# t-kychen/GaussianProcess-MCMC

Measured on NVIDIA B200. Metric: GP log-lik evals/sec (N=4096, batched chains), higher is better.
Workload: dtype f64

## Files before the change

### gaussianprocess-mcmc_b200/csrc/capi.cu

```cuda
#include "common.cuh"
#include "sequences.cuh"
#include "../../include/gpmc.h"

#include <stdarg.h>
#include <string.h>
#include <mutex>
#include <algorithm>
#include <vector>

namespace gpmc {

static thread_local char g_err[1024] = "";
static std::recursive_mutex g_api_mutex;
ApiLock::ApiLock() { g_api_mutex.lock(); }
ApiLock::~ApiLock() { g_api_mutex.unlock(); }
void set_error(const char *fmt, ...)
{
    va_list ap;
    va_start(ap, fmt);
    vsnprintf(g_err, sizeof(g_err), fmt, ap);
    va_end(ap);
}

struct EventPair { cudaEvent_t a, b; };
// ... 271 lines not shown
    if (failed.empty()) return 0;

    BatchView Bk{backup, (long long)N * ld, ld, nullptr, nullptr};
    { int rc0 = diag_stats(Bk, N, mean_dev, bad_dev, B, s); if (rc0) return rc0; }
    std::vector<double> mean(B);
    std::vector<int> bad(B);
    GPMC_CUDA_CHECK(cudaMemcpyAsync(mean.data(), mean_dev, B * sizeof(double), cudaMemcpyDeviceToHost, s));
    GPMC_CUDA_CHECK(cudaMemcpyAsync(bad.data(), bad_dev, B * sizeof(int), cudaMemcpyDeviceToHost, s));
    GPMC_CUDA_CHECK(cudaStreamSynchronize(s));
    std::vector<double> jit(B, 0.0);
    std::vector<int> todo;
    for (int i : failed) {
        if (bad[i]) info[i] = GPMC_INFO_NOT_PD;
        else { jit[i] = mean[i] * 1e-6; todo.push_back(i); }
    }
    for (int attempt = 0; attempt < 5 && !todo.empty(); ++attempt) {
        const int nf = (int)todo.size();
        GPMC_CUDA_CHECK(cudaMemcpyAsync(map_dev, todo.data(), nf * sizeof(int), cudaMemcpyHostToDevice, s));
        GPMC_CUDA_CHECK(cudaMemcpyAsync(jit_dev, jit.data(), B * sizeof(double), cudaMemcpyHostToDevice, s));
        BatchView Am{A_dev, (long long)N * ld, ld, map_dev, nullptr};
        restore_jitter_kernel<<<dim3(64, nf), 256, 0, s>>>(Am, backup, N, jit_dev);
        GPMC_LAUNCH_CHECK();
        for (int i : todo) info[i] = 0;
        GPMC_CUDA_CHECK(cudaMemcpyAsync(info_dev, info.data(), B * sizeof(int), cudaMemcpyHostToDevice, s));
        rc = potrf_sequence(Am, N, nf, info_dev, W, NB * NB, 0, zero_upper, s);
        if (rc) return rc;
        GPMC_CUDA_CHECK(cudaMemcpyAsync(info.data(), info_dev, B * sizeof(int), cudaMemcpyDeviceToHost, s));
        GPMC_CUDA_CHECK(cudaStreamSynchronize(s));
        std::vector<int> still;
        for (int i : todo) if (info[i] != 0) { still.push_back(i); jit[i] *= 10.0; }
        todo.swap(still);
    }
    for (int i : todo) info[i] = GPMC_INFO_NOT_PD;
    GPMC_CUDA_CHECK(cudaMemcpyAsync(info_dev, info.data(), B * sizeof(int), cudaMemcpyHostToDevice, s));
    GPMC_CUDA_CHECK(cudaStreamSynchronize(s));
    return 0;
}

int gpmc_loglik_batched(const double *x_dev, int N, int D, const double *g_dev, const double *hyp_dev, int B, int P,
                        int kind, int jitter_policy, double *loglik_dev, int *info_dev, void *ws_dev, size_t ws_bytes,
                        void *stream)
{
    GPMC_API_LOCK();
    cudaStream_t s = (cudaStream_t)stream;
    const int n_ell = (kind == GPMC_KIND_SE_ARD) ? D : 1;
    if (N <= 0 || D <= 0 || B < 0 || P != n_ell + 2) { set_error("loglik: bad shape N=%d D=%d B=%d P=%d kind=%d", N, D, B, P, kind); return GPMC_EINVAL; }
    if (B == 0) return 0;
    const LoglikLayout l = loglik_layout(N, B);
    if (!ws_dev || ws_bytes < l.fixed_bytes + l.per_item_bytes) {
        set_error("loglik: workspace %zu bytes cannot hold one item (%zu needed)", ws_bytes, l.fixed_bytes + l.per_item_bytes);
        return GPMC_ENOMEM;
    }
    char *wp = (char *)ws_dev;
    double *jit_dev = (double *)wp; wp += align_up((size_t)B * sizeof(double), 256);
    int *map_dev = (int *)wp; wp += align_up((size_t)B * sizeof(int), 256);
    int *band_dev = (int *)wp; wp += 256;
    double *xbox = (double *)wp;
    wp += align_up((size_t)32 * l.ld * sizeof(double), 256);
    const size_t wave_cap = std::min<size_t>((ws_bytes - l.fixed_bytes) / l.per_item_bytes, (size_t)MAX_BATCH_ITEMS);
    const int wave = (int)std::min<size_t>(wave_cap, (size_t)B);
    g_last_W = 0;
    g_last_waves = (B + wave - 1) / wave;
    { int rc0 = fill_int(info_dev, 0, B, s); if (rc0) return rc0; }

    if (wave < B && band_compact_allowed() && envelope_enabled() && band_enabled()) {
        const int nblk = env_blocks(N);
        const size_t wenv = align_up((size_t)B * nblk * sizeof(int), 256);
        char *cp = wp;
        int *w_all = (int *)cp; cp += wenv;
        int *env_all = (int *)cp; cp += wenv;
        const size_t room = ws_bytes - l.fixed_bytes;
        if (2 * wenv + 256 < room) {
            GPMC_CUDA_CHECK(cudaMemsetAsync(band_dev, 0, 2 * sizeof(int), s));
            int rc = launch_band_bound(x_dev, N, D, hyp_dev, P, n_ell, B, w_all, nblk, band_dev, xbox, s);
            if (rc) return rc;
            int bh[2] = {0, 0};
            GPMC_CUDA_CHECK(cudaMemcpyAsync(bh, band_dev, sizeof(bh), cudaMemcpyDeviceToHost, s));
            GPMC_CUDA_CHECK(cudaStreamSynchronize(s));
            const int Wc = (int)align_up((size_t)BAND_ROWS + (size_t)ENV_ROWS * bh[1], 16);
            const size_t per_item = (size_t)N * Wc * sizeof(double) + (size_t)l.ld * sizeof(double) + (size_t)NB * NB * sizeof(double);
            const size_t wave_c = std::min<size_t>((room - 2 * wenv - 256) / per_item, (size_t)MAX_BATCH_ITEMS);
            const int waves_c = wave_c > 0 ? (int)((B + wave_c - 1) / wave_c) : 0;
            const int nb_lo = waves_c > 0 ? B / waves_c : 0, nb_hi = waves_c > 0 ? (B + waves_c - 1) / waves_c : 0;
            if (Wc < l.ld && waves_c > 0 && waves_c < g_last_waves && potrf_compact_ok(N, nb_lo, 1) && potrf_compact_ok(N, nb_hi, 1)) {
                double *border = (double *)cp; cp += align_up((size_t)nb_hi * l.ld * sizeof(double), 256);
                double *Wsc = (double *)cp; cp += (size_t)nb_hi * NB * NB * sizeof(double);
                double *mats_c = (double *)cp;
                g_last_W = Wc;
                g_last_waves = waves_c;
                for (int wi = 0, s0 = 0; wi < waves_c; ++wi) {
                    const int nb = nb_lo + (wi < B % waves_c ? 1 : 0);
                    BatchView A{mats_c, (long long)N * Wc, Wc, nullptr, nullptr, Wc, N, border, l.ld};
                    const Envelope env{env_all + (size_t)s0 * nblk, nblk, N, bh[0]};
                    const Band band{w_all + (size_t)s0 * nblk, nblk, bh[1], 0};
                    const double *hyp_w = hyp_dev + (size_t)s0 * P;
                    const double *g_w = g_dev + (size_t)s0 * N;
                    int *info_w = info_dev + s0;
                    auto fill = [&](BatchView V, int nitems, const double *jit) -> int {
                        int rc = launch_cov_assemble(x_dev, N, D, hyp_w, P, n_ell, GPMC_ASM_ADD_S | GPMC_ASM_LOWER_ONLY, jit, V, nitems, s, env, band);
                        if (rc) return rc;
                        return border_set(V, N, g_w, N, nitems, s);
                    };
                    auto diag = [&](const double *h) { return host_diag_value(h, n_ell); };
                    rc = factor_wave(fill, diag, A, N, nb, hyp_w, P, info_w, Wsc, jit_dev, map_dev, jitter_policy, 1, s, 0, env);
                    if (rc) return rc;
                    if ((rc = border_finish(A, N, loglik_dev + s0, info_w, nb, s, 0))) return rc;
                    s0 += nb;
                }
                return 0;
            }
        }
    }

    double *mats = (double *)wp;
    double *W = (double *)(wp + (size_t)wave * l.mat_elems * sizeof(double));
    const Envelope env_ws{(int *)(W + (size_t)wave * NB * NB), env_blocks(N), N};
    int *band_w = env_ws.blk + (size_t)wave * env_blocks(N);
    ClearJoin clear{s};

    for (int s0 = 0; s0 < B; s0 += wave) {
        const int nb = std::min(wave, B - s0);
        const double *hyp_w = hyp_dev + (size_t)s0 * P;
        const double *g_w = g_dev + (size_t)s0 * N;
        int *info_w = info_dev + s0;
        BatchView A{mats, (long long)l.mat_elems, l.ld, nullptr, nullptr};
        const int fuse = potrf_fuse_auto(N, nb, 1);
        Envelope env = (envelope_enabled() && !fuse) ? env_ws : Envelope{};
        Band band{};
        int rc = 0;
        if (env.blk && band_enabled()) {
            const int mode = band_clear_mode();
            if (clear.pending) {
                GPMC_CUDA_CHECK(cudaStreamWaitEvent(s, clear.cs->done, 0));
                clear.pending = false;
            }
            GPMC_CUDA_CHECK(cudaMemsetAsync(band_dev, 0, 2 * sizeof(int), s));
            rc = launch_band_bound(x_dev, N, D, hyp_w, P, n_ell, nb, band_w, env_blocks(N), band_dev, xbox, s);
            if (rc) return rc;
            int bh[2] = {-1, 0};
            if (mode != 2 || (long long)nb * ((N + NB - 1) / NB) >= 1024) {
                GPMC_CUDA_CHECK(cudaMemcpyAsync(bh, band_dev, sizeof(bh), cudaMemcpyDeviceToHost, s));
                GPMC_CUDA_CHECK(cudaStreamSynchronize(s));
            }
            env.band = bh[0];
            band = Band{band_w, env_blocks(N), bh[1], mode == 2};
            if (mode == 1) {
                ClearStream *cs = clear.cs ? clear.cs : (clear.cs = clear_stream());
                if (!cs) { set_error("loglik: the band clear stream could not be created"); return GPMC_EINVAL; }
                GPMC_CUDA_CHECK(cudaEventRecord(cs->start, s));
                GPMC_CUDA_CHECK(cudaStreamWaitEvent(cs->s, cs->start, 0));
                BatchView Aw{mats, (long long)l.mat_elems, l.ld, nullptr, nullptr};
                if ((rc = launch_band_clear(Aw, N, band, nb, cs->s))) return rc;
                GPMC_CUDA_CHECK(cudaEventRecord(cs->done, cs->s));
                clear.pending = true;
            }
        }
        auto fill = [&](BatchView V, int nitems, const double *jit) -> int {
            int rc = launch_cov_assemble(x_dev, N, D, hyp_w, P, n_ell, GPMC_ASM_ADD_S | GPMC_ASM_LOWER_ONLY, jit, V, nitems, s, env, band);
            if (rc) return rc;
            return border_set(V, N, g_w, N, nitems, s);
        };
        auto diag = [&](const double *h) { return host_diag_value(h, n_ell); };
        rc = factor_wave(fill, diag, A, N, nb, hyp_w, P, info_w, W, jit_dev, map_dev, jitter_policy, 1, s, fuse, env);
        if (rc) return rc;
        rc = border_finish(A, N, loglik_dev + s0, info_w, nb, s, fuse);
        if (rc) return rc;
    }
    return 0;
}

struct HostPath {
    cudaStream_t stream = nullptr;
    void *dev = nullptr;  size_t dev_bytes = 0;
    void *ws = nullptr;   size_t ws_bytes = 0;
    void *pin = nullptr;  size_t pin_bytes = 0;
};
static HostPath g_hp;

static int ensure(void **p, size_t *have, size_t need, bool pinned)
{
    if (*have >= need) return 0;
    if (*p) { if (pinned) cudaFreeHost(*p); else cudaFree(*p); *p = nullptr; *have = 0; }
    cudaError_t e = pinned ? cudaMallocHost(p, need) : cudaMalloc(p, need);
    if (e != cudaSuccess) { set_error("allocation of %zu bytes failed: %s", need, cudaGetErrorString(e)); return (int)e; }
    *have = need;
    return 0;
}
// ... 147 lines not shown
```

### gaussianprocess-mcmc_b200/csrc/common.cuh

```cuda
#pragma once
#include <cuda_runtime.h>
#include <stdint.h>
#include <stdio.h>
#include <math.h>

namespace gpmc {

#ifndef GPMC_NB
#define GPMC_NB 128
#endif
constexpr int NB = GPMC_NB;
static_assert(NB == 64 || NB == 128, "panel width must be 64 or 128");
constexpr int MAX_ELL = 8;
constexpr int MAX_BATCH_ITEMS = 32768;

enum KernelClass { KC_ASSEMBLE = 0, KC_GEMM = 1, KC_POTF2 = 2, KC_TRSM = 3, KC_SOLVE = 4, KC_INV = 5, KC_SYRK_R = 6, KC_VEC = 7,
                   KC_CLEAR = 8, KC_GRAD = 9, KC_COUNT = 10 };

void set_error(const char *fmt, ...);
struct ApiLock { ApiLock(); ~ApiLock(); };
#define GPMC_API_LOCK() gpmc::ApiLock _gpmc_api_lock
void prof_begin(int kc, cudaStream_t s);
void prof_end(int kc, cudaStream_t s);

// ... 56 lines not shown
}
__host__ __device__ __forceinline__ long long view_border_stride(const BatchView &v) { return v.W ? v.border_stride : v.stride; }

constexpr int ENV_ROWS = 64;
struct Envelope {
    int *blk = nullptr;
    int ld = 0;
    int n = 0;
    int band = -1;
};

struct Band {
    const int *w = nullptr;
    int ld = 0;
    int width = 0;
    int clear = 0;
};
__host__ __device__ inline int env_blocks(int n) { return (n + ENV_ROWS - 1) / ENV_ROWS; }

__device__ __forceinline__ int env_first_col(const Envelope &e, int m, int r0, int r1)
{
    if (!e.blk || r1 > e.n || r1 <= r0) return 0;
    const int *p = e.blk + (size_t)m * e.ld;
    int k = 0x7fffffff;
    for (int r = r0 / ENV_ROWS; r <= (r1 - 1) / ENV_ROWS; ++r) k = min(k, p[r]);
    return k;
}


int launch_cov_assemble(const double *x, int N, int D, const double *hyp, int P, int n_ell, int flags,
                        const double *jitter, BatchView A, int B, cudaStream_t s, Envelope env = {}, Band band = {});
int launch_band_bound(const double *x, int N, int D, const double *hyp, int P, int n_ell, int B, int *w, int ldw,
                      int *band_out, double *xbox, cudaStream_t s);
int launch_band_clear(BatchView A, int N, Band band, int B, cudaStream_t s);

int launch_grad_contract(const double *x, int N, int D, const double *hyp, int P, int n_ell, const double *alpha, int ldv,
                         const double *W, int ldW, long long strideW, const int *band_w, int ldw, const int *info,
                         double *partial, double *grad, int B, cudaStream_t s);

struct Operand {
    const double *base;
    long long stride;
    int ld;
};
enum Epilogue {
    EPI_SUB = 0,
    EPI_SET = 1,
    EPI_NEGSET = 2,
    EPI_R = 3,
    EPI_ADD = 4
};
struct GemmArgs {
    BatchView C;
    Operand A, B;
    int cr0, cc0;
    int rows, cols;
    int ar0, br0;
    int k0, bk0;
    int klen;
    int lower_only;
    int k_follow_row;
    int epi;
    int skip_upper;
    int border_row;
    const double *svec;
    long long stride_s;
    Envelope env;
};
int launch_gemm(const GemmArgs &a, int B, int kclass, cudaStream_t s);
void set_gemm_config(int cfg);
bool gemm_honours_envelope();

int launch_potf2(BatchView A, int n, int j0, double *W, long long strideW, int *info, int zero_upper,
                 int B, cudaStream_t s);
int launch_potf2_lite(BatchView A, int n, int j0, double *W, long long strideW, int *info, int zero_upper,
                      int B, cudaStream_t s);
int launch_potf2_reg(BatchView A, int n, int j0, double *W, long long strideW, int *info, int zero_upper,
                     int B, cudaStream_t s);
int launch_potf2_flow(BatchView A, int n, int j0, double *W, long long strideW, int *info, int zero_upper,
                      int B, cudaStream_t s);
int launch_panel_fused_flow(BatchView A, int n, int n_rows, int j0, double *W, long long strideW, int *info, int zero_upper,
                            int B, cudaStream_t s);
int launch_panel_fused(BatchView A, int n, int n_rows, int j0, double *W, long long strideW, int *info, int zero_upper,
                       int B, cudaStream_t s);
void set_lookahead_mode(int mode);
void set_potrf_window(int w);
void set_potf2_mode(int mode);

int launch_trsm_panel(BatchView A, int n, int j0, const double *W, long long strideW, int B, cudaStream_t s);
int launch_trsm_panel8(BatchView A, int n, int j0, const double *W, long long strideW, int B, cudaStream_t s,
                       int row_start = -1, int n_mat = -1, Envelope env = {});
int launch_trmm_panel8(BatchView A, int rows, int c0, int width, const double *W, long long strideW, int B, cudaStream_t s);
int launch_inv_blocks8(BatchView A, int n, double *W, long long strideW, int B, cudaStream_t s);
void set_trsm_mode(int mode);
bool trsm_honours_envelope();
void set_trsm_blocks_per_cta(int v);

int launch_solve_reduce(BatchView L, int n, const double *a, const double *b, int ldv, double *zout,
                        double *loglik, const int *info, int B, cudaStream_t s);
int launch_quad_logdet(BatchView L, int n, const double *z, int ldv, double *loglik, const int *info, int B, cudaStream_t s);
int launch_trmv(BatchView T, int n, int upper, int mode, const double *x, const double *add, const double *svec,
                int ldv, double *out, int B, cudaStream_t s);

void set_sds_mode(int mode);
void set_panel_fuse(int mode);
void set_lookahead_split(int mode);
void set_inverse_window(int w);
void set_sds_literal(int v);
void set_sds_runahead(int r);
void set_sds_pin_schedule(int v);
void sds_loop_stats(long long *rounds, long long *idle_rounds, long long *ladders);

int run_fp64_peak(int which, int iters, double *tflops, double *ms);
int run_dmma_ilp(int nacc, int warps_per_sm, int iters, double *tflops);

}
```

### gaussianprocess-mcmc_b200/csrc/potf2_reg.cu

```cuda
#include "common.cuh"
#include "../../include/gpmc.h"

namespace gpmc {

static_assert(NB == 128, "potf2_reg is written for a panel width of 128 (16 x 16 fragments, 8 warps)");
constexpr int PR_NF = NB / 8;
constexpr int PR_WARPS = PR_NF / 2;
constexpr int PR_THREADS = PR_WARPS * 32;
constexpr int PR_SLOTS = PR_NF + 1;

__device__ __forceinline__ void dmma884_r(double &c0, double &c1, double a, double b)
{
    asm volatile("mma.sync.aligned.m8n8k4.row.col.f64.f64.f64.f64 {%0,%1}, {%2}, {%3}, {%0,%1};\n"
                 : "+d"(c0), "+d"(c1)
                 : "d"(a), "d"(b));
}

__device__ __forceinline__ double pivot_rsqrt(double a)
{
    double y;
    asm("rsqrt.approx.ftz.f64 %0, %1;" : "=d"(y) : "d"(a));
    const double h = 0.5 * a;
    const double e = fma(-(h * y), y, 0.5);
    return fma(y * e, fma(1.5, e, 1.0), y);
}
__device__ __forceinline__ double pivot_rcp(double a)
{
    double y;
    asm("rcp.approx.ftz.f64 %0, %1;" : "=d"(y) : "d"(a));
    const double e = fma(-a, y, 1.0);
    return fma(y, fma(e, e, e), y);
}

__device__ __forceinline__ void slot_rc(int s, int w, int &R, int &C, bool &isA)
{
    if (s < 2 * (w + 1)) { C = s >> 1; isA = (s & 1) == 0; }
    else { C = s - w - 1; isA = false; }
    R = isA ? w : PR_NF - 1 - w;
}

template <int S>
__device__ __forceinline__ void slot_update(double (&acc)[PR_SLOTS][2], int w, double xa0, double xa1, double xb0, double xb1,
                                            const double (*sX)[64], int frag_off)
{
    int R, C; bool isA;
    slot_rc(S, w, R, C, isA);
    const double n0 = isA ? -xa0 : -xb0, n1 = isA ? -xa1 : -xb1;
    double2 xc;
    if (C == R) xc = make_double2(-n0, -n1);
    else xc = *reinterpret_cast<const double2 *>(&sX[C][frag_off]);
    dmma884_r(acc[S][0], acc[S][1], n0, xc.x);
    dmma884_r(acc[S][0], acc[S][1], n1, xc.y);
}

#define PR_CASE(S) case S: slot_update<S>(acc, w, xa0, xa1, xb0, xb1, sX, frag_off);
#define PR_PICK(S) case S: p0 = acc[S][0]; p1 = acc[S][1]; break;
#define PR_PICK_ALL PR_PICK(0) PR_PICK(1) PR_PICK(2) PR_PICK(3) PR_PICK(4) PR_PICK(5) PR_PICK(6) PR_PICK(7) PR_PICK(8) \
    PR_PICK(9) PR_PICK(10) PR_PICK(11) PR_PICK(12) PR_PICK(13) PR_PICK(14) PR_PICK(15) PR_PICK(16)

__device__ __forceinline__ void pick_slot(const double (&acc)[PR_SLOTS][2], int slot, double &p0, double &p1)
{
    p0 = p1 = 0.0;
    switch (slot) { PR_PICK_ALL default: break; }
}

constexpr int PF_LC_ELEMS = (PR_NF * (PR_NF + 1) / 2) * 64;
constexpr int PF_SMEM = (PF_LC_ELEMS + PR_NF * 64) * (int)sizeof(double);

template <bool FUSED>
__global__ void __launch_bounds__(PR_THREADS, 2)
potf2_reg_kernel(BatchView A, int n, int j0, double *__restrict__ W, long long strideW, int *__restrict__ info, int zero_upper, int n_rows)
{
    extern __shared__ __align__(16) double pf_dyn[];
    double *Lc = pf_dyn;
    double *W8c = pf_dyn + PF_LC_ELEMS;
    __shared__ __align__(16) double sD[64];
    __shared__ __align__(16) double sL8[64], sW8[64];
    __shared__ __align__(16) double sX[PR_NF][64];
    __shared__ int s_fail;
    const int item = blockIdx.x;
    if (A.count && item >= *A.count) return;
    const int m = batch_item(A, item);
    double *Ab = view_elem(A, m, j0, j0);
    double *Wb = W + (size_t)m * strideW;
    const int ld = A.ld;
    const int nv = min(NB, n - j0);
    const int tid = threadIdx.x, w = tid >> 5, lane = tid & 31;
    const int fr = lane >> 2, fk = lane & 3;
    const int frag_off = fr * 8 + 2 * fk;
    const int rowA = w, rowB = PR_NF - 1 - w;

    if (tid == 0) s_fail = 0;
    double acc[PR_SLOTS][2];
#pragma unroll
    for (int s = 0; s < PR_SLOTS; ++s) {
        int R, C; bool isA;
        slot_rc(s, w, R, C, isA);
        const int gr = R * 8 + fr, gc = C * 8 + 2 * fk;
        double2 v = make_double2(0.0, 0.0);
        if (gr < nv && gc < nv) v = *reinterpret_cast<const double2 *>(Ab + (size_t)gr * ld + gc);
        if (gr >= nv || gc >= nv) v.x = (gr == gc) ? 1.0 : 0.0;
        if (gr >= nv || gc + 1 >= nv) v.y = (gr == gc + 1) ? 1.0 : 0.0;
        acc[s][0] = v.x;
        acc[s][1] = v.y;
    }
    double xa0 = 0.0, xa1 = 0.0, xb0 = 0.0, xb1 = 0.0;
    __syncthreads();

#pragma unroll 1
    for (int b = 0; b < PR_NF; ++b) {
        const bool own_diag = (b < PR_WARPS) ? (w == b) : (w == PR_NF - 1 - b);
        if (own_diag) {
            double d0, d1;
            pick_slot(acc, (b < PR_WARPS) ? 2 * b : PR_SLOTS - 1, d0, d1);
            *reinterpret_cast<double2 *>(&sD[frag_off]) = make_double2(d0, d1);
            __syncwarp();
            const int l16 = lane & 15, r8 = lane & 7;
            double v[8];
#pragma unroll
            for (int c = 0; c < 8; c += 2) {
                const double2 t = *reinterpret_cast<const double2 *>(&sD[r8 * 8 + c]);
                v[c] = (l16 < 8) ? ((c <= r8) ? t.x : 0.0) : ((c == r8) ? 1.0 : 0.0);
                v[c + 1] = (l16 < 8) ? ((c + 1 <= r8) ? t.y : 0.0) : ((c + 1 == r8) ? 1.0 : 0.0);
            }
            int fail = 0;
            double piv = __shfl_sync(0xffffffffu, v[0], 0);
#pragma unroll
            for (int c = 0; c < 8; ++c) {
                if (!(piv > 0.0) && fail == 0) fail = j0 + b * 8 + c + 1;
                const double pr = pivot_rcp(piv);
                const double rinv = pivot_rsqrt(piv);
                const double pnext = (c < 7) ? __shfl_sync(0xffffffffu, fma(-(v[c] * v[c]), pr, v[c + 1]), c + 1) : 0.0;
                v[c] = (l16 == c) ? piv * rinv : v[c] * rinv;
#pragma unroll
                for (int j = c + 1; j < 8; ++j) {
                    const double ljc = __shfl_sync(0xffffffffu, v[c], j);
                    v[j] = fma(-v[c], ljc, v[j]);
                }
                piv = pnext;
            }
            if (lane < 8) {
                const int gr = b * 8 + r8;
#pragma unroll
                for (int c = 0; c < 8; c += 2) {
                    const double2 lrow = make_double2((c <= r8) ? v[c] : 0.0, (c + 1 <= r8) ? v[c + 1] : 0.0);
                    *reinterpret_cast<double2 *>(&sL8[r8 * 8 + c]) = lrow;
                    if (FUSED) *reinterpret_cast<double2 *>(&Lc[(b * (b + 1) / 2 + b) * 64 + r8 * 8 + c]) = lrow;
                }
#pragma unroll
                for (int c = 0; c < 8; ++c)
                    if (c <= r8 && gr < nv) Ab[(size_t)gr * ld + b * 8 + c] = v[c];
                if (fail != 0 && lane == 0 && s_fail == 0) s_fail = fail;
            } else if (lane < 16) {
#pragma unroll
                for (int c = 0; c < 8; ++c) {
                    sW8[c * 8 + r8] = v[c];
                    if (FUSED) W8c[b * 64 + c * 8 + r8] = v[c];
                    Wb[(size_t)(b * 8 + c) * NB + b * 8 + r8] = v[c];
                }
            }
        }
        __syncthreads();
        {
            const int slotA = (b < w) ? 2 * b : -1;
            const int slotB = (b <= w) ? 2 * b + 1 : ((b < rowB) ? w + 1 + b : -1);
            if (slotB >= 0) {
                const double2 wv = *reinterpret_cast<const double2 *>(&sW8[frag_off]);
                const double2 lv = *reinterpret_cast<const double2 *>(&sL8[frag_off]);
                double a0, a1, b0, b1;
                pick_slot(acc, slotA, a0, a1);
                pick_slot(acc, slotB, b0, b1);
                double x0 = 0.0, x1 = 0.0, y0 = 0.0, y1 = 0.0;
                dmma884_r(x0, x1, a0, wv.x);
                dmma884_r(y0, y1, b0, wv.x);
                dmma884_r(x0, x1, a1, wv.y);
                dmma884_r(y0, y1, b1, wv.y);
                double r0 = a0, r1 = a1, q0 = b0, q1 = b1;
                dmma884_r(r0, r1, -x0, lv.x);
                dmma884_r(q0, q1, -y0, lv.x);
                dmma884_r(r0, r1, -x1, lv.y);
                dmma884_r(q0, q1, -y1, lv.y);
                dmma884_r(x0, x1, r0, wv.x);
                dmma884_r(y0, y1, q0, wv.x);
                dmma884_r(x0, x1, r1, wv.y);
                dmma884_r(y0, y1, q1, wv.y);
                xb0 = y0; xb1 = y1;
                *reinterpret_cast<double2 *>(&sX[rowB][frag_off]) = make_double2(y0, y1);
                if (FUSED) *reinterpret_cast<double2 *>(&Lc[(rowB * (rowB + 1) / 2 + b) * 64 + frag_off]) = make_double2(y0, y1);
                {
                    const int gr = rowB * 8 + fr, gc = b * 8 + 2 * fk;
                    if (gr < nv) {
                        if (gc + 1 < nv) *reinterpret_cast<double2 *>(Ab + (size_t)gr * ld + gc) = make_double2(y0, y1);
                        else if (gc < nv) Ab[(size_t)gr * ld + gc] = y0;
                    }
                }
                if (slotA >= 0) {
                    xa0 = x0; xa1 = x1;
                    *reinterpret_cast<double2 *>(&sX[rowA][frag_off]) = make_double2(x0, x1);
                    if (FUSED) *reinterpret_cast<double2 *>(&Lc[(rowA * (rowA + 1) / 2 + b) * 64 + frag_off]) = make_double2(x0, x1);
                    const int gr = rowA * 8 + fr, gc = b * 8 + 2 * fk;
                    if (gr < nv) {
                        if (gc + 1 < nv) *reinterpret_cast<double2 *>(Ab + (size_t)gr * ld + gc) = make_double2(x0, x1);
                        else if (gc < nv) Ab[(size_t)gr * ld + gc] = x0;
                    }
                }
            }
        }
        __syncthreads();
        {
            const int start = (b + 1 <= w) ? 2 * (b + 1) : w + b + 2;
            switch (start) {
                PR_CASE(0) PR_CASE(1) PR_CASE(2) PR_CASE(3) PR_CASE(4) PR_CASE(5) PR_CASE(6) PR_CASE(7) PR_CASE(8)
                PR_CASE(9) PR_CASE(10) PR_CASE(11) PR_CASE(12) PR_CASE(13) PR_CASE(14) PR_CASE(15) PR_CASE(16)
                default: break;
            }
        }
    }

    __syncthreads();
    if (tid == 0 && s_fail != 0) {
        if (info[m] == 0) info[m] = s_fail;
    }
    if (FUSED) {
        const int row_start = (j0 + NB < n) ? NB : n - j0;
        const int rows_end = n_rows - j0;
#pragma unroll 1
        for (int row0 = row_start; row0 < rows_end; row0 += 8 * PR_WARPS) {
            if (row0 + w * 8 >= rows_end) continue;
            const int r = row0 + w * 8 + fr;
            const bool rv = r < rows_end;
            double *grow = Ab + (size_t)min(r, rows_end - 1) * ld + 2 * fk;
            double t[PR_NF][2];
#pragma unroll
            for (int b8 = 0; b8 < PR_NF; ++b8) {
                double2 v = make_double2(0.0, 0.0);
                if (rv && b8 * 8 + 2 * fk < nv) v = *reinterpret_cast<const double2 *>(grow + b8 * 8);
                t[b8][0] = v.x;
                t[b8][1] = v.y;
            }
#pragma unroll
            for (int b8 = 0; b8 < PR_NF; ++b8) {
                const double2 wv = *reinterpret_cast<const double2 *>(&W8c[b8 * 64 + frag_off]);
                const double2 lv = *reinterpret_cast<const double2 *>(&Lc[(b8 * (b8 + 1) / 2 + b8) * 64 + frag_off]);
                double x0 = 0.0, x1 = 0.0;
                dmma884_r(x0, x1, t[b8][0], wv.x);
                dmma884_r(x0, x1, t[b8][1], wv.y);
                double r0 = t[b8][0], r1 = t[b8][1];
                dmma884_r(r0, r1, -x0, lv.x);
                dmma884_r(r0, r1, -x1, lv.y);
                dmma884_r(x0, x1, r0, wv.x);
                dmma884_r(x0, x1, r1, wv.y);
                const double nx0 = -x0, nx1 = -x1;
#pragma unroll
                for (int bp = b8 + 1; bp < PR_NF; ++bp) {
                    const double2 lp = *reinterpret_cast<const double2 *>(&Lc[(bp * (bp + 1) / 2 + b8) * 64 + frag_off]);
                    dmma884_r(t[bp][0], t[bp][1], nx0, lp.x);
                    dmma884_r(t[bp][0], t[bp][1], nx1, lp.y);
                }
                if (rv) {
                    const int c = b8 * 8 + 2 * fk;
                    if (c + 1 < nv) *reinterpret_cast<double2 *>(grow + b8 * 8) = make_double2(x0, x1);
                    else if (c < nv) grow[b8 * 8] = x0;
                }
            }
        }
    }
    if (zero_upper) {
        for (int e = tid; e < nv * nv; e += PR_THREADS) {
            const int r = e / nv, c = e - r * nv;
            if (c > r) Ab[(size_t)r * ld + c] = 0.0;
        }
    }
}

int launch_potf2_reg(BatchView A, int n, int j0, double *W, long long strideW, int *info, int zero_upper, int B, cudaStream_t s)
{
    if (B <= 0) return 0;
    if ((A.ld & 1) || (j0 & 1)) { set_error("potf2: ld=%d j0=%d must be even", A.ld, j0); return GPMC_EALIGN; }
    prof_begin(KC_POTF2, s);
    potf2_reg_kernel<false><<<B, PR_THREADS, 0, s>>>(A, n, j0, W, strideW, info, zero_upper, n);
    prof_end(KC_POTF2, s);
    GPMC_LAUNCH_CHECK();
    return 0;
}

int launch_panel_fused(BatchView A, int n, int n_rows, int j0, double *W, long long strideW, int *info, int zero_upper, int B, cudaStream_t s)
{
    if (B <= 0) return 0;
    if ((A.ld & 1) || (j0 & 1)) { set_error("panel: ld=%d j0=%d must be even", A.ld, j0); return GPMC_EALIGN; }
    if (A.W) { set_error("panel: the fused panel kernel does not take the compact band layout"); return GPMC_EINVAL; }
    static DeviceOnce attr_set;
    if (attr_set.first()) GPMC_CUDA_CHECK(cudaFuncSetAttribute(potf2_reg_kernel<true>, cudaFuncAttributeMaxDynamicSharedMemorySize, PF_SMEM));
    prof_begin(KC_POTF2, s);
    potf2_reg_kernel<true><<<B, PR_THREADS, PF_SMEM, s>>>(A, n, j0, W, strideW, info, zero_upper, n_rows);
    prof_end(KC_POTF2, s);
    GPMC_LAUNCH_CHECK();
    return 0;
}

}
```

### gaussianprocess-mcmc_b200/csrc/sequences.cu

```cuda
#include "sequences.cuh"
#include "../../include/gpmc.h"

#include <algorithm>

namespace gpmc {

__global__ void zero_upper_kernel(BatchView A, int n)
{
    const int b = blockIdx.z;
    if (A.count && b >= *A.count) return;
    const int m = batch_item(A, b);
    double *Ab = A.base + (size_t)m * A.stride;
    const int r = blockIdx.y * blockDim.y + threadIdx.y;
    const int c = blockIdx.x * blockDim.x + threadIdx.x;
    if (r < n && c < n && c > r) Ab[(size_t)r * A.ld + c] = 0.0;
}

__global__ void fill_int_kernel(int *p, int v, int n)
{
    const int i = blockIdx.x * blockDim.x + threadIdx.x;
    if (i < n) p[i] = v;
}
__global__ void fill_int_mapped_kernel(int *p, int v, const int *map, const int *count)
{
// ... 123 lines not shown
    GPMC_LAUNCH_CHECK();
    return 0;
}

static int sm_count()
{
    static int sms = 0;
    if (sms == 0) {
        int dev = 0;
        if (cudaGetDevice(&dev) != cudaSuccess || cudaDeviceGetAttribute(&sms, cudaDevAttrMultiProcessorCount, dev) != cudaSuccess || sms <= 0)
            sms = 148;
    }
    return sms;
}

static int g_schedule_batch = 0;
void set_schedule_batch(int B) { g_schedule_batch = B > 0 ? B : 0; }
static int schedule_batch(int B) { return g_schedule_batch > 0 ? g_schedule_batch : B; }

static int g_window_override = 0;
void set_potrf_window(int w) { g_window_override = (w > 0 && w % NB == 0) ? w : 0; }

static int potrf_window_for(int n, int B)
{
    const int nt = (n + 127) / 128;
    if (g_window_override) return g_window_override >= n ? 0 : g_window_override;
    if ((long long)B * nt >= 1024 && 2 * B > sm_count()) return 0;
    return n >= 12288 ? 1024 : 512;
}

static int g_trsm_mode = 0;
void set_trsm_mode(int mode) { g_trsm_mode = mode; }
bool trsm_honours_envelope() { return g_trsm_mode == 0; }
static int g_potf2_mode = 0;
void set_potf2_mode(int mode) { g_potf2_mode = mode; }
static bool lite_panels() { return g_trsm_mode == 0 && g_potf2_mode != 1; }


struct LookAhead {
    cudaStream_t panel = nullptr, inwin = nullptr;
    cudaEvent_t ev_q = nullptr, ev_p = nullptr, ev_a = nullptr;
    bool ok = false;
};
static LookAhead *lookahead_ctx()
{
    static LookAhead las[64];
    static bool tried_dev[64] = {};
    int dev = 0;
    if (cudaGetDevice(&dev) != cudaSuccess || dev < 0 || dev >= 64) return nullptr;
    LookAhead &la = las[dev];
    bool &tried = tried_dev[dev];
    if (!tried) {
        tried = true;
        int lo = 0, hi = 0;
        bool ok = cudaDeviceGetStreamPriorityRange(&lo, &hi) == cudaSuccess;
        ok = ok && cudaStreamCreateWithPriority(&la.panel, cudaStreamNonBlocking, hi) == cudaSuccess;
        ok = ok && cudaStreamCreateWithPriority(&la.inwin, cudaStreamNonBlocking, hi) == cudaSuccess;
        ok = ok && cudaEventCreateWithFlags(&la.ev_q, cudaEventDisableTiming) == cudaSuccess;
        ok = ok && cudaEventCreateWithFlags(&la.ev_p, cudaEventDisableTiming) == cudaSuccess;
        ok = ok && cudaEventCreateWithFlags(&la.ev_a, cudaEventDisableTiming) == cudaSuccess;
        la.ok = ok;
    }
    return la.ok ? &la : nullptr;
}
static int g_lookahead_mode = 0;
void set_lookahead_mode(int mode) { g_lookahead_mode = mode; }

static int g_split_mode = 0;
void set_lookahead_split(int mode) { g_split_mode = mode; }

static int g_panel_fuse = 0;
void set_panel_fuse(int mode) { g_panel_fuse = mode; }

int potrf_fuse_auto(int n, int B, int border_rows)
{
    B = schedule_batch(B);
    if (!lite_panels() || (g_potf2_mode != 0 && g_potf2_mode != 3) || g_panel_fuse == 1) return 0;
    if (g_panel_fuse == 2) return 1;
    if (n + border_rows <= 640) return 1;
    return (B >= 4 * sm_count() && n + border_rows <= 1664) ? 1 : 0;
}

static bool compact_kernels() { return NB == BAND_ROWS && g_trsm_mode == 0 && g_potf2_mode == 0; }
bool potrf_compact_ok(int n, int B, int border_rows)
{
    const int Bs = schedule_batch(B);
    return compact_kernels() && potrf_window_for(n, Bs) == 0 && g_lookahead_mode != 2 && !potrf_fuse_auto(n, B, border_rows);
}

int potrf_sequence(BatchView A, int n, int B, int *info, double *W, long long strideW, long long w_step,
                   int zero_upper_flag, cudaStream_t s, int border_rows, int fuse, Envelope env)
{
    if (A.W && (fuse || border_rows != 1 || w_step || zero_upper_flag || !env.blk || !compact_kernels())) {
        set_error("potrf_sequence: the compact band layout needs the envelope-aware kernels and one border row");
        return GPMC_EINVAL;
    }
    if (fuse && (!lite_panels() || (g_potf2_mode != 0 && g_potf2_mode != 3))) { set_error("potrf_sequence: fused panels need the default panel kernels"); return GPMC_EINVAL; }
    if (border_rows < 0) { set_error("potrf_sequence: border_rows < 0"); return GPMC_EINVAL; }
    const int nr = n + border_rows;
    const int xrows = border_rows > 1 ? border_rows : 0;
    const int brow = border_rows == 1 ? n : 0;
    const bool lite = lite_panels();
    const int Bs = schedule_batch(B);
    const int window = potrf_window_for(n, Bs);
    const Operand self{A.base, A.stride, A.ld};
    const int wlen = window > 0 ? window : n;
    LookAhead *la = nullptr;
    if (!fuse && n > 2 * NB && (g_lookahead_mode == 2 || (g_lookahead_mode == 0 && 2 * Bs <= sm_count()))) la = lookahead_ctx();
    const cudaStream_t sG = s;
    const cudaStream_t sQ = la ? (window > 0 ? la->inwin : s) : s;
    const cudaStream_t sP = la ? la->panel : s;

    auto update = [&](int j0, int width, int k_begin, int k_end, cudaStream_t st) -> int {
        GemmArgs g{};
        g.C = A; g.A = self; g.B = self;
        g.cr0 = j0; g.cc0 = j0; g.rows = n - j0 + xrows; g.cols = width;
        if (env.band >= 0 && xrows == 0) g.rows = std::min(g.rows, NB + env.band * ENV_ROWS);
        g.border_row = brow;
        g.ar0 = j0; g.br0 = j0; g.k0 = k_begin; g.bk0 = k_begin; g.klen = k_end - k_begin;
        g.epi = EPI_SUB;
        g.skip_upper = 1;
        g.env = env;
        return launch_gemm(g, B, KC_GEMM, st);
    };

    auto extra_rows_update = [&](int c0, int cols, int k_begin, int klen, cudaStream_t st) -> int {
        if (xrows == 0 || cols <= 0) return 0;
        GemmArgs g{};
        g.C = A; g.A = self; g.B = self;
        g.cr0 = n; g.cc0 = c0; g.rows = xrows; g.cols = cols;
        g.ar0 = n; g.br0 = c0; g.k0 = k_begin; g.bk0 = k_begin; g.klen = klen;
        g.epi = EPI_SUB;
        return launch_gemm(g, B, KC_GEMM, st);
    };

    for (int w0 = 0; w0 < n; w0 += wlen) {
        const int w1 = std::min(n, w0 + wlen);
        if (la && sQ != sG) {
            GPMC_CUDA_CHECK(cudaEventRecord(la->ev_a, sG));
            GPMC_CUDA_CHECK(cudaStreamWaitEvent(sQ, la->ev_a, 0));
            if (w0 > 0 && w1 < n) {
                GemmArgs g{};
                g.C = A; g.A = self; g.B = self;
                g.cr0 = w1; g.cc0 = w1; g.rows = n - w1; g.cols = n - w1;
                g.border_row = brow;
                g.ar0 = w1; g.br0 = w1; g.k0 = w0 - wlen; g.bk0 = w0 - wlen; g.klen = wlen;
                g.lower_only = 1;
                g.epi = EPI_SUB;
                g.skip_upper = 1;
                g.env = env;
                int rc = launch_gemm(g, B, KC_GEMM, sG);
                if (rc) return rc;
                if ((rc = extra_rows_update(w1, n - w1, w0 - wlen, wlen, sG))) return rc;
            }
        }
        const bool paired = w0 > 0 && w1 < n;
        const bool many_ctas = (long long)Bs * ((n - w0 + 127) / 128) * 2 >= 8LL * sm_count();
        const bool split_cols = la && (g_split_mode == 1 || paired || (g_split_mode == 0 && !many_ctas));
        for (int j0 = w0; j0 < w1; j0 += NB) {
            const int width = std::min(NB, n - j0);
            double *Wj = W + (size_t)(j0 / NB) * w_step;
            int rc;
            if (!la) {
                if (j0 > w0 && (rc = update(j0, width, w0, j0, s))) return rc;
            } else if (!split_cols) {
                if (j0 > w0) {
                    GPMC_CUDA_CHECK(cudaStreamWaitEvent(sQ, la->ev_p, 0));
                    if ((rc = update(j0, width, w0, j0, sQ))) return rc;
                }
                GPMC_CUDA_CHECK(cudaEventRecord(la->ev_q, sQ));
                GPMC_CUDA_CHECK(cudaStreamWaitEvent(sP, la->ev_q, 0));
            } else {
                if (j0 - NB > w0 && (rc = update(j0, width, w0, j0 - NB, sQ))) return rc;
                if (j0 > w0) {
                    GPMC_CUDA_CHECK(cudaStreamWaitEvent(sQ, la->ev_p, 0));
                    if ((rc = update(j0, width, j0 - NB, j0, sQ))) return rc;
                }
                GPMC_CUDA_CHECK(cudaEventRecord(la->ev_q, sQ));
                GPMC_CUDA_CHECK(cudaStreamWaitEvent(sP, la->ev_q, 0));
            }
            if (fuse) {
                if ((rc = (g_potf2_mode == 3 ? launch_panel_fused_flow(A, n, nr, j0, Wj, strideW, info, zero_upper_flag, B, sP)
                                             : launch_panel_fused(A, n, nr, j0, Wj, strideW, info, zero_upper_flag, B, sP)))) return rc;
                if (la) GPMC_CUDA_CHECK(cudaEventRecord(la->ev_p, sP));
                continue;
            }
            rc = !lite ? launch_potf2(A, n, j0, Wj, strideW, info, zero_upper_flag, B, sP)
                 : (g_potf2_mode == 2 ? launch_potf2_lite(A, n, j0, Wj, strideW, info, zero_upper_flag, B, sP)
                    : (g_potf2_mode == 3 ? launch_potf2_flow(A, n, j0, Wj, strideW, info, zero_upper_flag, B, sP)
                                         : launch_potf2_reg(A, n, j0, Wj, strideW, info, zero_upper_flag, B, sP)));
            if (rc) return rc;
            if (j0 + NB < n && (rc = (g_trsm_mode == 1 ? launch_trsm_panel(A, nr, j0, Wj, strideW, B, sP)
                                                        : launch_trsm_panel8(A, nr, j0, Wj, strideW, B, sP, -1, -1, env)))) return rc;
            if (j0 + NB >= n && xrows > 0 && (rc = launch_trsm_panel8(A, nr, j0, Wj, strideW, B, sP, n, n))) return rc;
            if (la) GPMC_CUDA_CHECK(cudaEventRecord(la->ev_p, sP));
        }
        if (la) GPMC_CUDA_CHECK(cudaStreamWaitEvent(sG, la->ev_p, 0));
        if (w1 < n) {
            const bool split = la && sQ != sG;
            const int w2 = std::min(n, w1 + wlen);
            GemmArgs g{};
            g.C = A; g.A = self; g.B = self;
            g.cr0 = w1; g.cc0 = w1; g.rows = n - w1 + (split ? xrows : 0); g.cols = split ? w2 - w1 : n - w1;
            g.border_row = brow;
            g.ar0 = w1; g.br0 = w1; g.k0 = w0; g.bk0 = w0; g.klen = w1 - w0;
            g.lower_only = split ? 0 : 1;
            g.epi = EPI_SUB;
            g.skip_upper = 1;
            g.env = env;
            int rc = launch_gemm(g, B, KC_GEMM, sG);
            if (rc) return rc;
            if (!split && (rc = extra_rows_update(w1, n - w1, w0, w1 - w0, sG))) return rc;
        }
    }
    if (zero_upper_flag) return zero_upper(A, n, B, s);
    return 0;
}

__global__ void border_set_kernel(BatchView A, int n, const double *__restrict__ rhs, int ldv, int len)
{
    const int b = blockIdx.y;
    if (A.count && b >= *A.count) return;
    const int m = batch_item(A, b);
    const int i = blockIdx.x * blockDim.x + threadIdx.x;
    if (i < len) *view_elem(A, m, n, i) = (i < n) ? rhs[(size_t)m * ldv + i] : 0.0;
}

int border_set(BatchView A, int n, const double *rhs, int ldv, int B, cudaStream_t s)
{
    if (B <= 0) return 0;
    const int len = A.W ? (int)A.border_stride : A.ld;
    prof_begin(KC_VEC, s);
    border_set_kernel<<<dim3((len + 255) / 256, B), 256, 0, s>>>(A, n, rhs, ldv, len);
    prof_end(KC_VEC, s);
    GPMC_LAUNCH_CHECK();
    return 0;
}

__global__ void border_get_kernel(BatchView A, int n, double *__restrict__ z, int ldv, const int *__restrict__ info)
{
    const int b = blockIdx.y;
    if (A.count && b >= *A.count) return;
    const int m = batch_item(A, b);
    const int i = blockIdx.x * blockDim.x + threadIdx.x;
    if (i < n) z[(size_t)m * ldv + i] = (info && info[m] != 0) ? nan("") : *view_elem(A, m, n, i);
}

int border_get(BatchView A, int n, double *z, int ldv, const int *info, int B, cudaStream_t s)
{
    if (B <= 0) return 0;
    prof_begin(KC_VEC, s);
    border_get_kernel<<<dim3((n + 255) / 256, B), 256, 0, s>>>(A, n, z, ldv, info);
    prof_end(KC_VEC, s);
    GPMC_LAUNCH_CHECK();
    return 0;
}

int border_finish(BatchView A, int n, double *loglik, const int *info, int B, cudaStream_t s, int solved)
{
    if (B <= 0) return 0;
    const long long bstride = view_border_stride(A);
    if (bstride > 0x7fffffffLL) { set_error("border_finish: item stride %lld does not fit the vector stride", bstride); return GPMC_EINVAL; }
    double *row = view_elem(A, 0, n, 0);
    if (solved) return loglik ? launch_quad_logdet(A, n, row, (int)bstride, loglik, info, B, s) : 0;
    const int j0 = (n - 1) / NB * NB;
    const int nv = n - j0;
// ... 120 lines not shown
```

### gaussianprocess-mcmc_b200/csrc/sequences.cuh

```cuda
#pragma once
#include "common.cuh"

#include <functional>

namespace gpmc {

int potrf_sequence(BatchView A, int n, int B, int *info, double *W, long long strideW, long long w_step,
                   int zero_upper, cudaStream_t s, int border_rows = 0, int fuse = 0, Envelope env = {});
int potrf_fuse_auto(int n, int B, int border_rows);
bool potrf_compact_ok(int n, int B, int border_rows);

int factor_wave(const std::function<int(BatchView, int, const double *)> &fill, const std::function<double(const double *)> &diag_value,
                BatchView A, int N, int nb, const double *hyp_w, int P, int *info_w, double *W, double *jit_dev, int *map_dev,
                int jitter_policy, int border_rows, cudaStream_t s, int fuse = 0, Envelope env = {}, long long w_step = 0);
bool envelope_enabled();
bool band_enabled();

int border_set(BatchView A, int n, const double *rhs, int ldv, int B, cudaStream_t s);
int border_finish(BatchView A, int n, double *loglik, const int *info, int B, cudaStream_t s, int solved = 0);
int border_get(BatchView A, int n, double *z, int ldv, const int *info, int B, cudaStream_t s);

int inverse_sequence(BatchView A, int n, int B, const double *W, long long strideW, cudaStream_t s);
void set_schedule_batch(int B);

int r_sequence(BatchView Rm, BatchView U, int n, int B, const double *svec, long long stride_s, cudaStream_t s);

size_t loglik_grad_workspace_bytes(int N, int D, int B);

int fill_int(int *p, int v, int n, cudaStream_t s);
int fill_int_mapped(int *p, int v, const int *map, const int *count, int nmax, cudaStream_t s);
int add_diag(BatchView A, int n, const double *jitter, int B, cudaStream_t s);
int diag_stats(BatchView A, int n, double *mean_out, int *nonpos_out, int B, cudaStream_t s);
int add_diag_vec(BatchView A, int n, const double *v, int ldv, int B, cudaStream_t s);
int zero_upper(BatchView A, int n, int B, cudaStream_t s);
int copy_rows(double *dst, int ldd, const double *src, int lds, int n, int rows, cudaStream_t s);

inline size_t align_up(size_t v, size_t a) { return (v + a - 1) / a * a; }
inline int ld_for(int n) { return (n + 15) / 16 * 16; }

}
```

Before: 37610.

## Enable fused panel factor+solve kernel for compact band layout with envelope skipping

Extends the fused POTF2+TRSM panel kernel so it handles the compact banded storage. It walks row blocks under the band, skips blocks whose envelope starts past the panel, and also solves the border row. The compact path no longer excludes cases where panel fusion would be chosen, and it now enables fusion by default. This removes separate TRSM launches per panel in the compact path, at the cost of more serialized work inside one kernel per matrix.

```diff
diff --git a/gaussianprocess-mcmc_b200/csrc/capi.cu b/gaussianprocess-mcmc_b200/csrc/capi.cu
--- a/gaussianprocess-mcmc_b200/csrc/capi.cu
+++ b/gaussianprocess-mcmc_b200/csrc/capi.cu
@@ -377,7 +377,7 @@
             const size_t wave_c = std::min<size_t>((room - 2 * wenv - 256) / per_item, (size_t)MAX_BATCH_ITEMS);
             const int waves_c = wave_c > 0 ? (int)((B + wave_c - 1) / wave_c) : 0;
             const int nb_lo = waves_c > 0 ? B / waves_c : 0, nb_hi = waves_c > 0 ? (B + waves_c - 1) / waves_c : 0;
-            if (Wc < l.ld && waves_c > 0 && waves_c < g_last_waves && potrf_compact_ok(N, nb_lo, 1) && potrf_compact_ok(N, nb_hi, 1)) {
+            if (Wc < l.ld && waves_c > 0 && waves_c < g_last_waves && potrf_compact_ok(N, nb_lo) && potrf_compact_ok(N, nb_hi)) {
                 double *border = (double *)cp; cp += align_up((size_t)nb_hi * l.ld * sizeof(double), 256);
                 double *Wsc = (double *)cp; cp += (size_t)nb_hi * NB * NB * sizeof(double);
                 double *mats_c = (double *)cp;
@@ -397,7 +397,7 @@
                         return border_set(V, N, g_w, N, nitems, s);
                     };
                     auto diag = [&](const double *h) { return host_diag_value(h, n_ell); };
-                    rc = factor_wave(fill, diag, A, N, nb, hyp_w, P, info_w, Wsc, jit_dev, map_dev, jitter_policy, 1, s, 0, env);
+                    rc = factor_wave(fill, diag, A, N, nb, hyp_w, P, info_w, Wsc, jit_dev, map_dev, jitter_policy, 1, s, potrf_fuse_compact(), env);
                     if (rc) return rc;
                     if ((rc = border_finish(A, N, loglik_dev + s0, info_w, nb, s, 0))) return rc;
                     s0 += nb;
diff --git a/gaussianprocess-mcmc_b200/csrc/common.cuh b/gaussianprocess-mcmc_b200/csrc/common.cuh
--- a/gaussianprocess-mcmc_b200/csrc/common.cuh
+++ b/gaussianprocess-mcmc_b200/csrc/common.cuh
@@ -162,7 +162,7 @@
 int launch_panel_fused_flow(BatchView A, int n, int n_rows, int j0, double *W, long long strideW, int *info, int zero_upper,
                             int B, cudaStream_t s);
 int launch_panel_fused(BatchView A, int n, int n_rows, int j0, double *W, long long strideW, int *info, int zero_upper,
-                       int B, cudaStream_t s);
+                       int B, cudaStream_t s, Envelope env = {});
 void set_lookahead_mode(int mode);
 void set_potrf_window(int w);
 void set_potf2_mode(int mode);
diff --git a/gaussianprocess-mcmc_b200/csrc/potf2_reg.cu b/gaussianprocess-mcmc_b200/csrc/potf2_reg.cu
--- a/gaussianprocess-mcmc_b200/csrc/potf2_reg.cu
+++ b/gaussianprocess-mcmc_b200/csrc/potf2_reg.cu
@@ -67,9 +67,49 @@
 constexpr int PF_LC_ELEMS = (PR_NF * (PR_NF + 1) / 2) * 64;
 constexpr int PF_SMEM = (PF_LC_ELEMS + PR_NF * 64) * (int)sizeof(double);
 
+__device__ __forceinline__ void fused_solve8(double *grow, bool rv, int nv, int b8s, const double *Lc, const double *W8c,
+                                             int frag_off, int fk)
+{
+    double t[PR_NF][2];
+#pragma unroll
+    for (int b8 = 0; b8 < PR_NF; ++b8) {
+        double2 v = make_double2(0.0, 0.0);
+        if (rv && b8 >= b8s && b8 * 8 + 2 * fk < nv) v = *reinterpret_cast<const double2 *>(grow + b8 * 8);
+        t[b8][0] = v.x;
+        t[b8][1] = v.y;
+    }
+#pragma unroll
+    for (int b8 = 0; b8 < PR_NF; ++b8) {
+        if (b8 < b8s) continue;
+        const double2 wv = *reinterpret_cast<const double2 *>(&W8c[b8 * 64 + frag_off]);
+        const double2 lv = *reinterpret_cast<const double2 *>(&Lc[(b8 * (b8 + 1) / 2 + b8) * 64 + frag_off]);
+        double x0 = 0.0, x1 = 0.0;
+        dmma884_r(x0, x1, t[b8][0], wv.x);
+        dmma884_r(x0, x1, t[b8][1], wv.y);
+        double r0 = t[b8][0], r1 = t[b8][1];
+        dmma884_r(r0, r1, -x0, lv.x);
+        dmma884_r(r0, r1, -x1, lv.y);
+        dmma884_r(x0, x1, r0, wv.x);
+        dmma884_r(x0, x1, r1, wv.y);
+        const double nx0 = -x0, nx1 = -x1;
+#pragma unroll
+        for (int bp = b8 + 1; bp < PR_NF; ++bp) {
+            const double2 lp = *reinterpret_cast<const double2 *>(&Lc[(bp * (bp + 1) / 2 + b8) * 64 + frag_off]);
+            dmma884_r(t[bp][0], t[bp][1], nx0, lp.x);
+            dmma884_r(t[bp][0], t[bp][1], nx1, lp.y);
+        }
+        if (rv) {
+            const int c = b8 * 8 + 2 * fk;
+            if (c + 1 < nv) *reinterpret_cast<double2 *>(grow + b8 * 8) = make_double2(x0, x1);
+            else if (c < nv) grow[b8 * 8] = x0;
+        }
+    }
+}
+
 template <bool FUSED>
 __global__ void __launch_bounds__(PR_THREADS, 2)
-potf2_reg_kernel(BatchView A, int n, int j0, double *__restrict__ W, long long strideW, int *__restrict__ info, int zero_upper, int n_rows)
+potf2_reg_kernel(BatchView A, int n, int j0, double *__restrict__ W, long long strideW, int *__restrict__ info, int zero_upper, int n_rows,
+                 Envelope env)
 {
     extern __shared__ __align__(16) double pf_dyn[];
     double *Lc = pf_dyn;
@@ -221,47 +261,30 @@
     if (tid == 0 && s_fail != 0) {
         if (info[m] == 0) info[m] = s_fail;
     }
-    if (FUSED) {
+    if (FUSED && !A.W) {
         const int row_start = (j0 + NB < n) ? NB : n - j0;
         const int rows_end = n_rows - j0;
 #pragma unroll 1
         for (int row0 = row_start; row0 < rows_end; row0 += 8 * PR_WARPS) {
             if (row0 + w * 8 >= rows_end) continue;
             const int r = row0 + w * 8 + fr;
-            const bool rv = r < rows_end;
-            double *grow = Ab + (size_t)min(r, rows_end - 1) * ld + 2 * fk;
-            double t[PR_NF][2];
-#pragma unroll
-            for (int b8 = 0; b8 < PR_NF; ++b8) {
-                double2 v = make_double2(0.0, 0.0);
-                if (rv && b8 * 8 + 2 * fk < nv) v = *reinterpret_cast<const double2 *>(grow + b8 * 8);
-                t[b8][0] = v.x;
-                t[b8][1] = v.y;
-            }
-#pragma unroll
-            for (int b8 = 0; b8 < PR_NF; ++b8) {
-                const double2 wv = *reinterpret_cast<const double2 *>(&W8c[b8 * 64 + frag_off]);
-                const double2 lv = *reinterpret_cast<const double2 *>(&Lc[(b8 * (b8 + 1) / 2 + b8) * 64 + frag_off]);
-                double x0 = 0.0, x1 = 0.0;
-                dmma884_r(x0, x1, t[b8][0], wv.x);
-                dmma884_r(x0, x1, t[b8][1], wv.y);
-                double r0 = t[b8][0], r1 = t[b8][1];
-                dmma884_r(r0, r1, -x0, lv.x);
-                dmma884_r(r0, r1, -x1, lv.y);
-                dmma884_r(x0, x1, r0, wv.x);
-                dmma884_r(x0, x1, r1, wv.y);
-                const double nx0 = -x0, nx1 = -x1;
-#pragma unroll
-                for (int bp = b8 + 1; bp < PR_NF; ++bp) {
-                    const double2 lp = *reinterpret_cast<const double2 *>(&Lc[(bp * (bp + 1) / 2 + b8) * 64 + frag_off]);
-                    dmma884_r(t[bp][0], t[bp][1], nx0, lp.x);
-                    dmma884_r(t[bp][0], t[bp][1], nx1, lp.y);
-                }
-                if (rv) {
-                    const int c = b8 * 8 + 2 * fk;
-                    if (c + 1 < nv) *reinterpret_cast<double2 *>(grow + b8 * 8) = make_double2(x0, x1);
-                    else if (c < nv) grow[b8 * 8] = x0;
-                }
+            fused_solve8(Ab + (size_t)min(r, rows_end - 1) * ld + 2 * fk, r < rows_end, nv, 0, Lc, W8c, frag_off, fk);
+        }
+    }
+    if (FUSED && A.W && j0 + NB < n) {
+        const int r_first = j0 + NB;
+        const int nmb = (n - r_first + 63) / 64;
+        const int nbl = (env.band >= 0 && env.band < nmb - 1) ? env.band : nmb;
+#pragma unroll 1
+        for (int rb = 0; rb <= nbl; ++rb) {
+            const int row0 = r_first + rb * 64;
+            if (rb < nbl) {
+                const int e = env_first_col(env, m, row0, min(row0 + 64, n));
+                if (e >= j0 + NB || row0 + w * 8 >= n) continue;
+                const int r = min(row0 + w * 8 + fr, n - 1);
+                fused_solve8(view_elem(A, m, r, j0 + 2 * fk), row0 + w * 8 + fr < n, nv, max(e - j0, 0) / 8, Lc, W8c, frag_off, fk);
+            } else if (w == 0) {
+                fused_solve8(view_elem(A, m, n, j0 + 2 * fk), fr == 0, nv, 0, Lc, W8c, frag_off, fk);
             }
         }
     }
@@ -278,21 +301,22 @@
     if (B <= 0) return 0;
     if ((A.ld & 1) || (j0 & 1)) { set_error("potf2: ld=%d j0=%d must be even", A.ld, j0); return GPMC_EALIGN; }
     prof_begin(KC_POTF2, s);
-    potf2_reg_kernel<false><<<B, PR_THREADS, 0, s>>>(A, n, j0, W, strideW, info, zero_upper, n);
+    potf2_reg_kernel<false><<<B, PR_THREADS, 0, s>>>(A, n, j0, W, strideW, info, zero_upper, n, Envelope{});
     prof_end(KC_POTF2, s);
     GPMC_LAUNCH_CHECK();
     return 0;
 }
 
-int launch_panel_fused(BatchView A, int n, int n_rows, int j0, double *W, long long strideW, int *info, int zero_upper, int B, cudaStream_t s)
+int launch_panel_fused(BatchView A, int n, int n_rows, int j0, double *W, long long strideW, int *info, int zero_upper, int B, cudaStream_t s,
+                       Envelope env)
 {
     if (B <= 0) return 0;
     if ((A.ld & 1) || (j0 & 1)) { set_error("panel: ld=%d j0=%d must be even", A.ld, j0); return GPMC_EALIGN; }
-    if (A.W) { set_error("panel: the fused panel kernel does not take the compact band layout"); return GPMC_EINVAL; }
+    if (A.W && (!env.blk || n_rows != n + 1)) { set_error("panel: the compact band layout needs its envelope and one border row"); return GPMC_EINVAL; }
     static DeviceOnce attr_set;
     if (attr_set.first()) GPMC_CUDA_CHECK(cudaFuncSetAttribute(potf2_reg_kernel<true>, cudaFuncAttributeMaxDynamicSharedMemorySize, PF_SMEM));
     prof_begin(KC_POTF2, s);
-    potf2_reg_kernel<true><<<B, PR_THREADS, PF_SMEM, s>>>(A, n, j0, W, strideW, info, zero_upper, n_rows);
+    potf2_reg_kernel<true><<<B, PR_THREADS, PF_SMEM, s>>>(A, n, j0, W, strideW, info, zero_upper, n_rows, env);
     prof_end(KC_POTF2, s);
     GPMC_LAUNCH_CHECK();
     return 0;
diff --git a/gaussianprocess-mcmc_b200/csrc/sequences.cu b/gaussianprocess-mcmc_b200/csrc/sequences.cu
--- a/gaussianprocess-mcmc_b200/csrc/sequences.cu
+++ b/gaussianprocess-mcmc_b200/csrc/sequences.cu
@@ -229,16 +229,17 @@
 }
 
 static bool compact_kernels() { return NB == BAND_ROWS && g_trsm_mode == 0 && g_potf2_mode == 0; }
-bool potrf_compact_ok(int n, int B, int border_rows)
+bool potrf_compact_ok(int n, int B)
 {
     const int Bs = schedule_batch(B);
-    return compact_kernels() && potrf_window_for(n, Bs) == 0 && g_lookahead_mode != 2 && !potrf_fuse_auto(n, B, border_rows);
-}
+    return compact_kernels() && potrf_window_for(n, Bs) == 0 && g_lookahead_mode != 2;
+}
+int potrf_fuse_compact() { return g_panel_fuse == 1 ? 0 : 1; }
 
 int potrf_sequence(BatchView A, int n, int B, int *info, double *W, long long strideW, long long w_step,
                    int zero_upper_flag, cudaStream_t s, int border_rows, int fuse, Envelope env)
 {
-    if (A.W && (fuse || border_rows != 1 || w_step || zero_upper_flag || !env.blk || !compact_kernels())) {
+    if (A.W && (border_rows != 1 || w_step || zero_upper_flag || !env.blk || !compact_kernels())) {
         set_error("potrf_sequence: the compact band layout needs the envelope-aware kernels and one border row");
         return GPMC_EINVAL;
     }
@@ -328,7 +329,7 @@
             }
             if (fuse) {
                 if ((rc = (g_potf2_mode == 3 ? launch_panel_fused_flow(A, n, nr, j0, Wj, strideW, info, zero_upper_flag, B, sP)
-                                             : launch_panel_fused(A, n, nr, j0, Wj, strideW, info, zero_upper_flag, B, sP)))) return rc;
+                                             : launch_panel_fused(A, n, nr, j0, Wj, strideW, info, zero_upper_flag, B, sP, A.W ? env : Envelope{})))) return rc;
                 if (la) GPMC_CUDA_CHECK(cudaEventRecord(la->ev_p, sP));
                 continue;
             }
diff --git a/gaussianprocess-mcmc_b200/csrc/sequences.cuh b/gaussianprocess-mcmc_b200/csrc/sequences.cuh
--- a/gaussianprocess-mcmc_b200/csrc/sequences.cuh
+++ b/gaussianprocess-mcmc_b200/csrc/sequences.cuh
@@ -8,7 +8,8 @@
 int potrf_sequence(BatchView A, int n, int B, int *info, double *W, long long strideW, long long w_step,
                    int zero_upper, cudaStream_t s, int border_rows = 0, int fuse = 0, Envelope env = {});
 int potrf_fuse_auto(int n, int B, int border_rows);
-bool potrf_compact_ok(int n, int B, int border_rows);
+bool potrf_compact_ok(int n, int B);
+int potrf_fuse_compact();
 
 int factor_wave(const std::function<int(BatchView, int, const double *)> &fill, const std::function<double(const double *)> &diag_value,
                 BatchView A, int N, int nb, const double *hyp_w, int P, int *info_w, double *W, double *jit_dev, int *map_dev,
```

Result: faster. 41180, median of 6 (+9.5%).
